# perdoch/hesaff

Measured on AMD Instinct MI355X. Metric: keypoints/sec (descriptors written), 4K grayscale batch, higher is better.
Workload: dtype f32

## Files before the change

hesaff_amd/csrc/capi_impl.h:

```cpp
#pragma once

namespace {

int fail(hesaff_ctx *c, const HsError &e)
{
   if (c) c->err = e.msg; else g_create_error = e.msg;
   return e.code;
}

#define HS_API_BEGIN try {
#define HS_API_END(ctx)                                              \
   }                                                                 \
   catch (const HsError &e) { return fail(ctx, e); }                 \
   catch (const std::exception &e) { return fail(ctx, HsError(HESAFF_ERR_NOMEM, e.what())); } \
   return HESAFF_OK;

void bind_device(hesaff_ctx *c) { HIP_TRY(hipSetDevice(c->device)); }

bool finite_f(float v) { return v == v && v - v == 0.0f; }

void validate_params(const hesaff_params &p)
{
   if (!finite_f(p.threshold) || !finite_f(p.edgeEigenValueRatio) || !finite_f(p.initialSigma) || !finite_f(p.convergenceThreshold) ||
       !finite_f(p.mrSize) || !finite_f(p.maxBinValue))
// ... 113 lines not shown
      if (const char *ov = getenv("HESAFF_OVERLAP")) c->no_overlap = atoi(ov) == 0;
      c->debug = getenv("HESAFF_DEBUG") != nullptr;
#endif
   } catch (const HsError &e) {
      hesaff_destroy(c);
      return fail(nullptr, e);
   } catch (const std::exception &e) {
      hesaff_destroy(c);
      return fail(nullptr, HsError(HESAFF_ERR_NOMEM, e.what()));
   }
   *out = c;
   return HESAFF_OK;
}

void hesaff_destroy(hesaff_ctx *c)
{
   if (!c) return;
   (void)hipSetDevice(c->device);
   if (c->stream) { (void)hipStreamSynchronize(c->stream); }
   DevBuf *bufs[] = {&c->t_smm, &c->t_sift, &c->t_bin0, &c->t_bin1, &c->t_w0, &c->t_w1, &c->t_pyr_taps, &c->t_patch_taps,
                     &c->t_patch_off, &c->t_patch_k, &c->b_gray, &c->b_up, &c->b_L, &c->b_L3, &c->b_R, &c->b_map, &c->b_bitmask, &c->b_prefix,
                     &c->b_blocksums, &c->b_generic, &c->b_counters, &c->b_cand, &c->b_rec_f, &c->b_rec_i, &c->b_rec_w, &c->b_hess_f, &c->b_hess_i,
                     &c->b_aff, &c->b_pw, &c->b_bins, &c->b_rank, &c->b_desc, &c->b_out, &c->b_starts, &c->b_patches,
                     &c->b_stage, &c->b_input, &c->t_mask_idx, &c->t_sgrad_nb, &c->t_sgrad_om, &c->t_vo_rows, &c->t_vo_src, &c->b_rowprefix, &c->b_trows, &c->b_trows2, &c->b_trows3,
                     &c->b_ex_len, &c->b_ex_sums, &c->b_ex_off, &c->b_ex_imgoff, &c->b_ex_starts, &c->b_jcoef[0], &c->b_jcoef[1], &c->b_jplane};
   for (DevBuf *b : bufs) b->release();
   for (hipEvent_t e : c->ev_pool) (void)hipEventDestroy(e);
   {
      hipStream_t all[6] = {c->side_streams[0], c->side_streams[1], c->side_streams[2], c->side_streams[3], c->sift_stream, c->aff_stream};
      for (int i = 0; i < 6; i++) {
         bool seen = all[i] == nullptr || all[i] == c->stream;
         for (int j = 0; j < i; j++) seen = seen || all[j] == all[i];
         if (!seen) (void)hipStreamSynchronize(all[i]);
      }
      for (int i = 0; i < HS_NSIDE; i++) if (c->ev_join[i]) (void)hipEventDestroy(c->ev_join[i]);
   }
   if (c->ev_fork) (void)hipEventDestroy(c->ev_fork);
   if (c->ev_detect_done) (void)hipEventDestroy(c->ev_detect_done);
   if (c->ev_batch_done) (void)hipEventDestroy(c->ev_batch_done);
   for (hipEvent_t e : c->ev_aff) (void)hipEventDestroy(e);
   for (int i = 0; i < HS_NSLOT; i++) {
      if (c->ev_extract_done[i]) (void)hipEventDestroy(c->ev_extract_done[i]);
      if (c->ev_sift_done[i]) (void)hipEventDestroy(c->ev_sift_done[i]);
      c->b_patches2[i].release();
   }
   c->b_siftvec2.release(); c->b_meanvar2.release(); c->b_siftvo2.release();
   if (c->h2d_stream) (void)hipStreamSynchronize(c->h2d_stream);
// ... 749 lines not shown
   Lists s = make_lists(c);
   hipStream_t st = c->stream;
   HIP_TRY(hipMemcpy2DAsync(c->gray.p, (size_t)c->gray.pitch * 4, img, (size_t)cols * 4, (size_t)cols * 4, rows, hipMemcpyHostToDevice, st));
   std::vector<float> x(n), y(n), sc(n);
   std::vector<int32_t> meta(n, 0), P0(n), alive(n);
   for (int i = 0; i < n; i++) { x[i] = kp[3 * i]; y[i] = kp[3 * i + 1]; sc[i] = kp[3 * i + 2]; }
   HIP_TRY(hipMemcpyAsync(s.hl.x, x.data(), (size_t)n * 4, hipMemcpyHostToDevice, st));
   HIP_TRY(hipMemcpyAsync(s.hl.y, y.data(), (size_t)n * 4, hipMemcpyHostToDevice, st));
   HIP_TRY(hipMemcpyAsync(s.hl.s, sc.data(), (size_t)n * 4, hipMemcpyHostToDevice, st));
   HIP_TRY(hipMemcpyAsync(s.hl.meta, meta.data(), (size_t)n * 4, hipMemcpyHostToDevice, st));
   HIP_TRY(hipMemcpyAsync(s.pw.A, A, (size_t)n * 16, hipMemcpyHostToDevice, st));
   HIP_TRY(hipMemsetAsync(s.counters, 0, 64 * 4, st));
   uint32_t nn = (uint32_t)n;
   HIP_TRY(hipMemcpyAsync(s.counters + 3, &nn, 4, hipMemcpyHostToDevice, st));
   hipLaunchKernelGGL(k_prepare_patch_given_A, dim3((n + 255) / 256), dim3(256), 0, st, s.hl, (const uint32_t *)(s.counters + 3), rows, cols,
                      c->consts, c->tables, s.pw);
   c->b_patches.ensure((size_t)n * HS_PATCH_PIX * 4);
   HIP_TRY(hipMemsetAsync(c->b_patches.p, 0, (size_t)n * HS_PATCH_PIX * 4, st));
   unsigned long long large_rows = 0;
   c->batch_max_p = 0;
   for (int i = 0; i < n; i++) {
      const float mrScale = ceilf(sc[i] * c->consts.mrSize);
      const long long P = (mrScale < 1.0e6f) ? 2 * (long long)mrScale + 3 : 0;
      if (P > HS_BIN3_PMAX && P <= c->max_p0 + 2) { large_rows += (unsigned long long)P; c->batch_max_p = std::max(c->batch_max_p, (int)P); }
   }
   if (large_rows > 0xffffffffull) throw HsError(HESAFF_ERR_NOMEM, "too many huge windows in one call");
   run_patch_stage(c, s, c->gray, c->b_patches.as<float>(), 0, (uint32_t)large_rows);
   uint32_t ovf = 0;
   HIP_TRY(hipMemcpyAsync(&ovf, s.counters + 6, 4, hipMemcpyDeviceToHost, st));
   HIP_TRY(hipMemcpyAsync(alive.data(), s.pw.alive, (size_t)n * 4, hipMemcpyDeviceToHost, st));
   if (patches) HIP_TRY(hipMemcpyAsync(patches, c->b_patches.p, (size_t)n * HS_PATCH_PIX * 4, hipMemcpyDeviceToHost, st));
   HIP_TRY(hipStreamSynchronize(st));
   HIP_TRY(hipGetLastError());
   if (ovf) throw HsError(HESAFF_ERR_NOMEM, "large-window row buffer exceeded (internal bound violated)");
   if (rejected) for (int i = 0; i < n; i++) rejected[i] = alive[i] ? 0 : 1;
   HS_API_END(c)
}

int hesaff_stage_sift(hesaff_ctx *c, int n, const float *patches, uint8_t *desc)
{
   if (!c || !patches || !desc || n < 0) return HESAFF_ERR_ARG;
   HS_API_BEGIN
   bind_device(c);
   if (n == 0) return HESAFF_OK;
   const size_t N = (size_t)n;
   const size_t off_alive = N * HS_PATCH_PIX * 4, off_mv = off_alive + N * 4, off_vec = off_mv + N * 8, off_desc = off_vec + N * 128 * 4;
   const size_t off_vo = (off_desc + N * 128 + 63) & ~(size_t)63, total = off_vo + N * HS_VO_PITCH * 8 + 64;
// ... 178 lines not shown
```

hesaff_amd/csrc/kernels_keypoint.h:

```cpp
#pragma once
#include <type_traits>
#include "device_common.h"
#include "kernels_pyramid.h"

struct PlaneTab {
   DPlane L[HS_MAX_OCTAVES][HS_NSCALES];
};

struct KpTables {
   const float *smm_mask;
   const float *sift_mask;
   const int32_t *mask_idx;
   int n_masked;
   const int4 *sgrad_nb;
   const int2 *sgrad_om;
   const int4 *vo_rows;
   const uint16_t *vo_src;
   const int32_t *bin0, *bin1;
   const float *w0, *w1;
   const float *patch_taps;
   const int32_t *patch_tap_off;
   const int32_t *patch_tap_k;
   int max_p0;
};
// ... 204 lines not shown
   hs_affine_groups(
      h_lo, n, tb.smm_mask, k, out, [&](uint32_t h) {
      const int meta = hl.meta[h];
      const int b = meta >> 8, octave = (meta >> 4) & 15, level = (meta >> 2) & 3;
      const DPlane &P = pt.L[octave][level];
      AffKp q;
      q.blur = P.img(b); q.rows = P.rows; q.cols = P.cols; q.pitch = P.pitch;
      q.x = hl.x[h]; q.y = hl.y[h]; q.s = hl.s[h]; q.pd = k.pd0 * (float)(1 << octave);
      return q;
   });
}

__global__ __launch_bounds__(64) void k_affine_stage(DPlane P, const float *__restrict__ kp , int n, KpTables tb, DConsts k,
                                                     AffineOut out)
{
   hs_affine_groups(0u, (uint32_t)n, tb.smm_mask, k, out, [&](uint32_t h) {
      AffKp q;
      q.blur = P.img(0); q.rows = P.rows; q.cols = P.cols; q.pitch = P.pitch;
      q.x = kp[4 * h]; q.y = kp[4 * h + 1]; q.s = kp[4 * h + 2]; q.pd = kp[4 * h + 3];
      return q;
   });
}

#define HS_NBINS 5
#define HS_BIN3_PMAX 512
__host__ __device__ inline int hs_patch_bin(int P) { return P <= 41 ? 0 : (P <= 64 ? 1 : (P <= 128 ? 2 : (P <= HS_BIN3_PMAX ? 3 : 4))); }

struct PatchWork {
   float *A;
   int32_t *P0;
   int32_t *alive;
   uint32_t *bin_count;
   uint32_t *bin_work;
   uint32_t *bin_items;
   uint32_t cap;
};

__device__ __forceinline__ int hs_window_p0(float s, float mrSize)
{
   const float mrScale = ceilf(s * mrSize);
   const int m = (mrScale < 1.0e6f) ? (int)mrScale : 1000000;
   return 2 * m + 1;
}

__global__ __launch_bounds__(256) void k_image_large_rows(HessList hl, const uint32_t *__restrict__ n_ptr, float mrSize, uint32_t *__restrict__ rows, int nimg);

template <bool RECTIFY>
__device__ __forceinline__ void hs_prepare_patch_body(const HessList &hl, uint32_t h_lo, uint32_t n, const AffineOut &aff, int imRows, int imCols,
                                                      const DConsts &k, const KpTables &tb, const PatchWork &pw)
// ... 165 lines not shown
```

hesaff_amd/csrc/kernels_patch.h:

```cpp
#pragma once
#include <type_traits>
#include "kernels_keypoint.h"

#define HS_PATCH_ARR 1684
#define HS_PATCH_PIX_IT 7
#define HS_NEED 82

struct PatchIO {
   DPlane image;
   float *patches;
   uint32_t h_base;
   float *trows;
   const uint32_t *row_prefix;
   uint32_t trows_cap;
   uint32_t *overflow;
};

__device__ __forceinline__ float hs_tap_inside(const HsPlaneBuf &im, float wx, float wy)
{
   const uint32_t off = ((uint32_t)(int)wy * im.pitch + (uint32_t)(int)wx) * 4u;
   wx = __builtin_amdgcn_fractf(wx);
   wy = __builtin_amdgcn_fractf(wy);
   const hs_v2u r0 = __builtin_amdgcn_raw_buffer_load_b64(im.rsrc, (int)off, 0, 0);
   const hs_v2u r1 = __builtin_amdgcn_raw_buffer_load_b64(im.rsrc, (int)off, (int)im.pitch_bytes, 0);
// ... 361 lines not shown
         }
      }
   }
   pa = da;
   pb = db;
}

template <bool PADDED>
__device__ __forceinline__ void hs_resample_reduced_batched(const float *__restrict__ T, int P, float scale, hs_row_taps taps, int r,
                                                            float *s_patch)
{
   const float c0 = (float)(P >> 1);
   for (int idx = threadIdx.x; idx < HS_PATCH_PIX; idx += 256) {
      const int jj = hs_div_small(idx, 1.0f / (float)HS_PATCH), ii = idx - jj * HS_PATCH;
      const int j = jj - (HS_PATCH >> 1), i = ii - (HS_PATCH >> 1);
      const float rx = c0 + (float)j * 0.0f, ry = c0 + (float)j * scale;
      float wx = rx + (float)i * scale, wy = ry + (float)i * 0.0f;
      const float fx = floorf(wx), fy = floorf(wy);
      wx -= fx; wy -= fy;
      const int y0 = min(max((int)fy, 0), P - 2);
      v2f pa, pb;
      hs_colpass4_rows<8, !PADDED>(T, y0, 2 * ii, P - 1, taps, r, pa, pb);
      s_patch[idx] = (1.0f - wy) * ((1.0f - wx) * pa.x + wx * pa.y) + (wy) * ((1.0f - wx) * pb.x + wx * pb.y);
   }
}

__device__ __forceinline__ void hs_resample_chunked(const float *__restrict__ T, int P, float scale, hs_row_taps taps, int r,
                                                    float *__restrict__ s_chunk, int chunk_rows, float *s_patch)
{
   const int tid = threadIdx.x;
   const float c0 = (float)(P >> 1);
   auto y0_of = [&](int jj) {
      const float wy = c0 + (float)(jj - (HS_PATCH >> 1)) * scale;
      return min(max((int)floorf(wy), 0), P - 2);
   };
   for (int jj0 = 0; jj0 < HS_PATCH;) {
      const int ylo = y0_of(jj0) - r;
      int jj1 = jj0;
      while (jj1 + 1 < HS_PATCH && y0_of(jj1 + 1) + r + 2 - ylo <= chunk_rows) jj1++;
      const int nrows = y0_of(jj1) + r + 2 - ylo;
      {
         const v2f *src = reinterpret_cast<const v2f *>(T + ylo * HS_NEED);
         v2f *dst = reinterpret_cast<v2f *>(s_chunk);
         const int n2 = nrows * (HS_NEED / 2);
#pragma unroll 4
         for (int i = tid; i < n2; i += 256) dst[i] = src[i];
      }
      __syncthreads();
      for (int idx = jj0 * HS_PATCH + tid; idx < (jj1 + 1) * HS_PATCH; idx += 256) {
         const int jj = hs_div_small(idx, 1.0f / (float)HS_PATCH), ii = idx - jj * HS_PATCH;
         const int j = jj - (HS_PATCH >> 1), i = ii - (HS_PATCH >> 1);
         const float rx = c0 + (float)j * 0.0f, ry = c0 + (float)j * scale;
         float wx = rx + (float)i * scale, wy = ry + (float)i * 0.0f;
         const float fx = floorf(wx), fy = floorf(wy);
         wx -= fx; wy -= fy;
         const int y0 = min(max((int)fy, 0), P - 2);
         const float *tc = s_chunk + (y0 - ylo) * HS_NEED + 2 * ii;
         auto ld = [&](int dy) { return *reinterpret_cast<const v2f *>(tc + dy * HS_NEED); };
         const v2f q0 = ld(0), q1 = ld(1);
         const float kc = taps[r];
         v2f da = kc * q0, db = kc * q1;
         v2f pj = q1, mj = q0;
#pragma unroll 4
         for (int jt = 1; jt <= r; jt++) {
            const v2f pn = ld(jt + 1), mn = ld(-jt);
            const float kj = taps[r + jt];
            const v2f sa = pj + mn, sb = pn + mj;
            da += kj * sa;
            db += kj * sb;
            pj = pn;
            mj = mn;
         }
         s_patch[idx] = (1.0f - wy) * ((1.0f - wx) * da.x + wx * da.y) + (wy) * ((1.0f - wx) * db.x + wx * db.y);
      }
      __syncthreads();
      jj0 = jj1 + 1;
   }
}

template <int NR, int NB>
__device__ __forceinline__ void hs_gather_slots(const HsPlaneBuf &img, const v2f *rc, const v2f *__restrict__ ctab, float a11, float a21, int half,
                                                int xb, int P, int r, float *__restrict__ srow, int sstride)
{
   const int lane = threadIdx.x & 63, pm = P - 1;
   float v[NR][NB];
#pragma unroll
   for (int it = 0; it < NB; it++) {
      const int xx = min(xb + lane + 64 * it, pm);
      const v2f c = ctab ? ctab[xx] : hs_col_coord(a11, a21, xx - half);
#pragma unroll
      for (int i = 0; i < NR; i++) {
         const v2f w = rc[i] + c;
         v[i][it] = hs_tap_inside(img, w.x, w.y);
      }
   }
#pragma unroll
// ... 137 lines not shown
         a1 = sA[jt + 1]; b1 = sB[jt + 1];
         tA0 += k * a0; tA1 += k * a1;
         tB0 += k * b0; tB1 += k * b1;
      }
      tA2.x = tA0; tA2.y = tA1; tB2.x = tB0; tB2.y = tB1;
      const int yA = rowA ? yy1 : yy0, yB = rowB == 2 ? yy2 : yy1;
      v2f *oA = reinterpret_cast<v2f *>(rowA ? out1 : out0) + colA;
      v2f *oB = reinterpret_cast<v2f *>(rowB == 2 ? out2 : out1) + colB;
      *oA = tA2;
      if (64 + lane < 3 * HS_PATCH) *oB = tB2;
      if (pad_r > 0) {
         if (yA == 0) for (int jr = 1; jr <= pad_r; jr++) oA[-jr * (HS_NEED / 2)] = tA2;
         if (yA == pm) for (int jr = 1; jr <= pad_r; jr++) oA[jr * (HS_NEED / 2)] = tA2;
         if (64 + lane < 3 * HS_PATCH) {
            if (yB == 0) for (int jr = 1; jr <= pad_r; jr++) oB[-jr * (HS_NEED / 2)] = tB2;
            if (yB == pm) for (int jr = 1; jr <= pad_r; jr++) oB[jr * (HS_NEED / 2)] = tB2;
         }
      }
   }
   HS_WAVE_LDS_SYNC();
}

#define HS_MID_PMAX 128
#define HS_MID_SROW 160
#define HS_BIG_SROW 640
#define HS_BIG_TAPS 128
#define HS_MID_RPAD 14
#define HS_BIG_RPAD 57
#define HS_CHUNK_MIN_ROWS 4
#define HS_MID_NIT3_BIG 2
#define HS_MID_NIT3_SMALL 1
#define HS_MID_BLOCKS (256 * 7)
#define HS_BIG_BLOCKS (256 * 8)

template <int PMAX> struct MidGeom {
   static constexpr bool BIG = PMAX > HS_MID_PMAX;
   static constexpr int SROW = BIG ? HS_BIG_SROW : HS_MID_SROW;
   static constexpr int NTAP = BIG ? HS_BIG_TAPS : 32;
   static constexpr int RPAD = BIG ? HS_BIG_RPAD : HS_MID_RPAD;
   static constexpr int CHUNK_MIN = BIG ? 0 : 64;
   static constexpr int SROWS = 12 * SROW > CHUNK_MIN * HS_NEED ? 12 * SROW : CHUNK_MIN * HS_NEED;
   static constexpr int CHUNK_ROWS = SROWS / HS_NEED;
   static constexpr int FLOATS = HS_PATCH_ARR + NTAP + 2 * (PMAX + 2) + SROWS;
};

template <int PMAX>
__global__ __launch_bounds__(256) void k_patch_mid(HessList hl, PatchWork pw, PatchIO io, KpTables tb)
{
   typedef MidGeom<PMAX> GM;
   constexpr int BIN = GM::BIG ? 3 : 2;
   constexpr int NIT = GM::BIG ? 4 : 2;
   constexpr int NIT3 = GM::BIG ? HS_MID_NIT3_BIG : HS_MID_NIT3_SMALL;
   extern __shared__ __attribute__((aligned(16))) float smem[];
   float *s_patch = smem;
   v2f *s_C = reinterpret_cast<v2f *>(s_patch + HS_PATCH_ARR + GM::NTAP);
   float *s_srow = reinterpret_cast<float *>(s_C + (PMAX + 2));
   float *Tp = io.trows + (size_t)blockIdx.x * ((size_t)(PMAX + 2 * GM::RPAD) * HS_NEED);

   const int tid = threadIdx.x, wave = tid >> 6;
   const uint32_t cnt = min(pw.bin_count[BIN], pw.cap);
   const int imPitch = io.image.pitch;

   __shared__ uint32_t s_item;
   for (;;) {
      if (tid == 0) s_item = atomicAdd(pw.bin_work + BIN, 1u);
      __syncthreads();
      const uint32_t wi = (uint32_t)__builtin_amdgcn_readfirstlane((int)s_item);
      if (wi >= cnt) break;
      const uint32_t h = pw.bin_items[(size_t)BIN * pw.cap + wi];
      const int b = hl.meta[h] >> 8;
      const HsPlaneBuf ib = hs_plane_buf(io.image.img(b), io.image.rows, imPitch);
      const float x = hl.x[h], y = hl.y[h];
      const float a11 = pw.A[4 * h], a12 = pw.A[4 * h + 1], a21 = pw.A[4 * h + 2], a22 = pw.A[4 * h + 3];
      const int P0 = pw.P0[h], P = P0 + 2, half = P >> 1;
      const float scale = (float)P0 / (float)HS_PATCH;
      const int K = tb.patch_tap_k[(P0 - 1) >> 1];
      const float *taps_g = tb.patch_taps + tb.patch_tap_off[(P0 - 1) >> 1];
      const hs_row_taps ktap = HS_ROW_TAPS(taps_g);
      for (int m = tid; m < P; m += 256) s_C[m] = hs_col_coord(a11, a21, m - half);
      __syncthreads();
      float *srowA = s_srow + wave * 3 * GM::SROW, *srowB = srowA + GM::SROW;
#pragma unroll 1
      for (int yy = wave; yy < P; yy += 12) {
         const int rr = K >> 1;
         if (yy + 8 < P)
            hs_row_stream3<NIT3>(ib, x, y, a12, a22, P, yy, yy + 4, yy + 8, scale, s_C, ktap, K, srowA, GM::SROW,
                                 Tp + (size_t)(yy + rr) * HS_NEED, Tp + (size_t)(yy + 4 + rr) * HS_NEED, Tp + (size_t)(yy + 8 + rr) * HS_NEED, rr);
         else if (yy + 4 < P)
            hs_row_stream2<NIT>(ib, x, y, a12, a22, P, yy, yy + 4, scale, s_C, ktap, K, srowA, srowB,
                                Tp + (size_t)(yy + (K >> 1)) * HS_NEED, Tp + (size_t)(yy + 4 + (K >> 1)) * HS_NEED, K >> 1);
         else
            hs_row_stream<NIT>(ib, x, y, a11, a12, a21, a22, P, yy, scale, s_C, ktap, K, srowA,
                               Tp + (size_t)(yy + (K >> 1)) * HS_NEED, K >> 1);
      }
      __syncthreads();
      if ((float)(K + 1) + (float)(HS_CHUNK_MIN_ROWS - 1) * scale <= (float)GM::CHUNK_ROWS)
         hs_resample_chunked(Tp + (K >> 1) * HS_NEED, P, scale, ktap, K >> 1, s_srow, GM::CHUNK_ROWS, s_patch);
      else
         hs_resample_reduced_batched<true>(Tp + (K >> 1) * HS_NEED, P, scale, ktap, K >> 1, s_patch);
      __syncthreads();
      for (int i = tid; i < HS_PATCH_PIX; i += 256) {
         float *po = io.patches + (size_t)(h - io.h_base) * HS_PATCH_PIX + i;
         hs_store_nt(po, s_patch[i]);
      }
      __syncthreads();
   }
}

#define HS_LARGE_CHUNK 18
#define HS_LARGE_NIT3 2

__global__ __launch_bounds__(256) void k_patch_large_rows(HessList hl, PatchWork pw, PatchIO io, KpTables tb, int srow_stride, int tap_stride, int nrow,
                                                          int p_lo, int p_hi)
{
   extern __shared__ __attribute__((aligned(16))) float smem[];
   const int wave = __builtin_amdgcn_readfirstlane((int)(threadIdx.x >> 6));
   float *srow = smem + (size_t)wave * (nrow * srow_stride + tap_stride);
   const uint32_t *pre = io.row_prefix;
   const uint32_t n_items = min(pw.bin_count[HS_NBINS - 1], pw.cap);
   if (n_items == 0) return;
   const uint32_t row_hi = pre[n_items];
   if (row_hi > io.trows_cap) {
      if (threadIdx.x == 0 && blockIdx.x == 0) *io.overflow = 1u;
      return;
   }
   const int imPitch = io.image.pitch;
   const uint32_t ntasks = (row_hi + HS_LARGE_CHUNK - 1) / HS_LARGE_CHUNK;
// ... 130 lines not shown
```

hesaff_amd/csrc/pipeline.hip:

```cpp
#include <hip/hip_runtime.h>
#include <algorithm>
#include <atomic>
#include <chrono>
#include <cmath>
#include <cstdio>
#include <cstdlib>
#include <cstring>
#include <string>
#include <vector>
#include <condition_variable>
#include <deque>
#include <future>
#include <map>
#include <memory>
#include <mutex>
#include <thread>

#include "../../include/hesaff_amd.h"
#include "host_tables.h"
#include "kernels_keypoint.h"
#include "kernels_patch.h"
#include "kernels_sift.h"
#include "kernels_pyramid.h"
#include "kernels_export.h"
// ... 106 lines not shown
      if (p) (void)hipFree(p);
      p = nullptr;
      bytes = 0;
   }
   template <class T> T *as() const { return (T *)p; }
};

struct OctGeom {
   int rows, cols, pitch;
   long long word_base;
   int words_per_row;
};

static inline int round_up(int v, int m) { return (v + m - 1) / m * m; }

#define HS_NSIDE 4
#define HS_LARGE_NW 2
#define HS_LARGE_SPLIT 1280
#define HS_AFF_BLOCKS_PER_CU 8
#define HS_GRID_LOC 1024
#define HS_GRID_DED 512
#define HS_GRID_SCAT 1024
#define HS_GRID_PACK 3584
#define HS_MID_CAP 6
#define HS_BIG_CAP 4
#define HS_OVERSUB 128u
#define HS_NSLOT 3
struct StreamSet { hipStream_t comp[4] = {nullptr, nullptr, nullptr, nullptr}; hipStream_t h2d = nullptr, d2h = nullptr; };
static std::mutex g_sets_mu;
static std::map<int, std::vector<StreamSet>> g_idle_sets;
static bool take_stream_set(int device, StreamSet &out)
{
   std::lock_guard<std::mutex> lk(g_sets_mu);
   std::vector<StreamSet> &v = g_idle_sets[device];
   if (v.empty()) return false;
   out = v.back();
   v.pop_back();
   return true;
}
static void give_stream_set(int device, const StreamSet &s)
{
   std::lock_guard<std::mutex> lk(g_sets_mu);
   g_idle_sets[device].push_back(s);
}

struct hesaff_ctx {
   hesaff_params par;
   int device = 0;
// ... 117 lines not shown
   hipStream_t h2d_stream = nullptr, d2h_stream = nullptr;
   hipEvent_t ev_exp[2][4] = {{nullptr, nullptr, nullptr, nullptr}, {nullptr, nullptr, nullptr, nullptr}};
   float export_ms = 0.0f; int32_t export_rows = 0;
   hipEvent_t ev_h2d[2] = {nullptr, nullptr}, ev_in_free[2] = {nullptr, nullptr}, ev_out_ready[2] = {nullptr, nullptr}, ev_d2h[2] = {nullptr, nullptr};
   struct HostSmall {
      void *p = nullptr; size_t bytes = 0;
      void *ensure(size_t need)
      {
         if (need > bytes) {
            if (p) (void)hipHostFree(p);
            p = nullptr; bytes = 0;
            const size_t cap = std::max<size_t>(need * 2, 4096);
            if (hipHostMalloc(&p, cap, hipHostMallocDefault) != hipSuccess) { p = nullptr; throw HsError(HESAFF_ERR_NOMEM, "hipHostMalloc failed (small result block)"); }
            bytes = cap;
         }
         return p;
      }
      void release() { if (p) (void)hipHostFree(p); p = nullptr; bytes = 0; }
   } h_small_end, h_small_mid, h_small_exp;
   struct HStarts {
      int32_t *q = nullptr;
      int32_t *data() const { return q; }
   } h_starts;
   DevBuf t_mask_idx, t_sgrad_nb, t_sgrad_om, t_vo_rows, t_vo_src, b_rowprefix, b_trows, b_trows2, b_trows3;
   DevBuf b_jcoef[2], b_jplane;
   DevBuf b_ex_len, b_ex_sums, b_ex_off, b_ex_imgoff, b_ex_starts;
   size_t rows_lds_set = 0;
   int n_cu = 256;
   uint32_t g_small0 = 256 * 6, g_small1 = 256 * 4, g_mid = HS_MID_BLOCKS, g_big = HS_BIG_BLOCKS, g_lfin = 256 * 4, g_shist = 256 * 32;
   uint32_t sgrad_grid = 256 * 32;
   uint32_t trows_rows = 4u << 20;

   hesaff_timings tm;
   int profiling = 0;
   int out_format = HESAFF_OUT_TEXT;
   int resume = 0;
   int pool_priority = -1;
   int stage_threads = 4;
   hipStream_t side_streams[HS_NSIDE] = {nullptr, nullptr, nullptr, nullptr};
   hipStream_t sift_stream = nullptr;
   hipStream_t aff_stream = nullptr;
   hipEvent_t ev_detect_done = nullptr, ev_batch_done = nullptr;
   std::vector<hipEvent_t> ev_aff;
   hipEvent_t ev_extract_done[HS_NSLOT] = {}, ev_sift_done[HS_NSLOT] = {};
   DevBuf b_patches2[HS_NSLOT];
   DevBuf b_siftvec2, b_meanvar2, b_siftvo2;
   hipEvent_t ev_fork = nullptr, ev_join[HS_NSIDE] = {nullptr, nullptr, nullptr, nullptr};
   bool fast_pyramid = false;
   bool no_overlap = false;
   bool debug = false;

   std::vector<hipEvent_t> ev_pool;
// ... 120 lines not shown
   t.bin0 = c->t_bin0.as<int32_t>(); t.bin1 = c->t_bin1.as<int32_t>();
   t.w0 = c->t_w0.as<float>(); t.w1 = c->t_w1.as<float>();
   t.patch_taps = c->t_patch_taps.as<float>(); t.patch_tap_off = c->t_patch_off.as<int32_t>(); t.patch_tap_k = c->t_patch_k.as<int32_t>();
   t.max_p0 = c->max_p0;
   t.mask_idx = c->t_mask_idx.as<int32_t>();
   t.sgrad_nb = c->t_sgrad_nb.as<int4>(); t.sgrad_om = c->t_sgrad_om.as<int2>();
   t.vo_rows = c->t_vo_rows.as<int4>(); t.vo_src = c->t_vo_src.as<uint16_t>();
   t.n_masked = c->n_masked;
}

DPlane make_plane(float *p, int rows, int cols, int pitch)
{
   DPlane d;
   d.p = p; d.rows = rows; d.cols = cols; d.pitch = pitch; d.img_stride = (long long)rows * pitch;
   return d;
}

template <class KERNEL> void set_dyn_lds(KERNEL kern, size_t lds)
{
   HIP_TRY(hipFuncSetAttribute((const void *)kern, hipFuncAttributeMaxDynamicSharedMemorySize, (int)lds));
}

size_t small_extract_lds_bytes(int bin) { return (size_t)(bin == 0 ? SmallGeom<0>::FLOATS : SmallGeom<1>::FLOATS) * 4; }
size_t mid_lds_bytes() { return (size_t)MidGeom<HS_MID_PMAX>::FLOATS * 4; }
size_t big_lds_bytes() { return (size_t)MidGeom<HS_BIN3_PMAX>::FLOATS * 4; }

constexpr size_t HS_LDS_PER_CU = 160 * 1024;
struct LargeGeom { int srow_stride, tap_stride; size_t lds; };
LargeGeom large_geom(int pmax)
{
   LargeGeom g;
   g.srow_stride = round_up((int)(pmax * 1.23) + 16, 64);
   g.tap_stride = round_up((int)(pmax * 0.22) + 8, 64);
   g.lds = (size_t)4 * (g.srow_stride + g.tap_stride) * 4;
   return g;
}

template <class KERNEL> uint32_t resident_grid(hesaff_ctx *c, KERNEL kern, int threads, size_t dyn_lds, uint32_t fallback_per_cu)
{
   int nb = 0;
   if (hipOccupancyMaxActiveBlocksPerMultiprocessor(&nb, (const void *)kern, threads, dyn_lds) != hipSuccess || nb < 1) {
      (void)hipGetLastError();
      nb = (int)fallback_per_cu;
   }
   return (uint32_t)c->n_cu * (uint32_t)nb;
}

void set_kernel_attrs(hesaff_ctx *c)
{
   set_dyn_lds(k_patch_extract_small<0>, small_extract_lds_bytes(0));
   set_dyn_lds(k_patch_extract_small<1>, small_extract_lds_bytes(1));
   set_dyn_lds(k_patch_mid<HS_MID_PMAX>, mid_lds_bytes());
   set_dyn_lds(k_patch_mid<HS_BIN3_PMAX>, big_lds_bytes());
   hipDeviceProp_t prop;
   HIP_TRY(hipGetDeviceProperties(&prop, c->device));
   c->n_cu = std::max(1, prop.multiProcessorCount);
   c->g_small0 = resident_grid(c, k_patch_extract_small<0>, 256, small_extract_lds_bytes(0), 6);
   c->g_small1 = resident_grid(c, k_patch_extract_small<1>, 256, small_extract_lds_bytes(1), 4);
   c->g_mid = std::min<uint32_t>(resident_grid(c, k_patch_mid<HS_MID_PMAX>, 256, mid_lds_bytes(), HS_MID_CAP), HS_MID_BLOCKS);
   c->g_big = std::min<uint32_t>(resident_grid(c, k_patch_mid<HS_BIN3_PMAX>, 256, big_lds_bytes(), HS_BIG_CAP), HS_BIG_BLOCKS);
   c->g_lfin = resident_grid(c, k_patch_large_finish, 256, 0, 4);
   c->g_shist = resident_grid(c, k_sift_hist, 64, 0, 32);
   c->sgrad_grid = (uint32_t)c->n_cu * 32u;
   c->g_small0 *= HS_OVERSUB; c->g_small1 *= HS_OVERSUB; c->g_shist *= HS_OVERSUB;
}

void plan_buffers(hesaff_ctx *c, int B, int H, int W);
void plan(hesaff_ctx *c, int B, int H, int W)
{
   try {
      plan_buffers(c, B, H, W);
   } catch (const HsError &e) {
      if (e.code == HESAFF_ERR_NOMEM) {
         DevBuf *bufs[] = {&c->b_gray, &c->b_up, &c->b_L, &c->b_L3, &c->b_R, &c->b_map, &c->b_bitmask, &c->b_prefix, &c->b_blocksums, &c->b_cand,
                           &c->b_rec_f, &c->b_rec_i, &c->b_rec_w, &c->b_hess_f, &c->b_hess_i, &c->b_aff, &c->b_pw, &c->b_bins, &c->b_rank, &c->b_desc,
                           &c->b_out, &c->b_starts};
         (void)hipStreamSynchronize(c->stream);
         for (DevBuf *b : bufs) b->release();
         c->map_clean = false;
      }
      throw;
   }
}
// ... 68 lines not shown
   c->b_counters.ensure(64 * 4);
   {
      const unsigned long long waves0 = (unsigned long long)((PW + EXM_STRIP - 1) / EXM_STRIP) * (unsigned long long)(PH / 32 + 1) * (unsigned long long)B;
      const unsigned long long cc = (unsigned long long)cap + (unsigned long long)cap / 8 + HS_CAND_BLOCK * waves0;
      if (cc > 0xfffffff0ull) throw HsError(HESAFF_ERR_ARG, "batch too large for 32-bit candidate indices");
      c->cand_cap = (uint32_t)cc;
      c->b_cand.ensure((size_t)cc * sizeof(CandRec));
   }
   c->b_rec_f.ensure(cap * 4 * 4);
   c->b_rec_i.ensure(cap * 4 * 4);
   c->b_rec_w.ensure(cap * 8);
   c->b_hess_f.ensure(cap * 4 * 4);
   c->b_hess_i.ensure(cap * 2 * 4);
   c->b_aff.ensure(cap * 6 * 4);
   c->b_pw.ensure(cap * 6 * 4);
   c->b_bins.ensure(cap * HS_NBINS * 4);
   c->b_rank.ensure((cap + 1) * 4);
   c->b_desc.ensure(cap * 128);
   c->b_out.ensure(cap * sizeof(KeyRec));
   c->b_starts.ensure(((size_t)(B + 1) * 3 + 2) * 4);
   const int max_p0 = (int)std::floor(std::sqrt((double)W * (double)H)) + 3;
   ensure_patch_taps(c, max_p0);
   refresh_tables_struct(c);
   c->b_trows2.ensure((size_t)HS_MID_BLOCKS * (HS_MID_PMAX + 2 * HS_MID_RPAD) * HS_NEED * 4);
   c->b_trows3.ensure((size_t)HS_BIG_BLOCKS * (HS_BIN3_PMAX + 2 * HS_BIG_RPAD) * HS_NEED * 4);
   {
      const LargeGeom lg = large_geom(c->max_p0 + 2);
      if (lg.lds / 4 > HS_LDS_PER_CU) throw HsError(HESAFF_ERR_ARG, "image too large for the large-window row kernel (sqrt(width x height) above about 27900)");
      const size_t want = std::min<size_t>(lg.lds + (size_t)8 * lg.srow_stride * 4, HS_LDS_PER_CU);
      if (want > c->rows_lds_set) {
         set_dyn_lds(k_patch_large_rows, want);
         c->rows_lds_set = want;
      }
   }
   c->B = B; c->H = H; c->W = W;
}

template <class LOAD> void exclusive_scan(hesaff_ctx *c, LOAD load, long long n, uint32_t *out, uint32_t *total)
{
   if (n <= 0) { HIP_TRY(hipMemsetAsync(total, 0, 4, c->stream)); return; }
   const int nb = (int)((n + SCAN_BLOCK - 1) / SCAN_BLOCK);
   uint32_t *bs = c->b_blocksums.as<uint32_t>();
   hipLaunchKernelGGL(k_scan_reduce<LOAD>, dim3(nb), dim3(256), 0, c->stream, load, n, bs);
   hipLaunchKernelGGL(k_scan_sums, dim3(1), dim3(256), 0, c->stream, bs, nb, total);
   hipLaunchKernelGGL(k_scan_down<LOAD>, dim3(nb), dim3(256), 0, c->stream, load, n, bs, out);
}

struct StageTimer {
// ... 117 lines not shown
   io.h_base = h_base;
   if (c->fast_pyramid && pt) {
      hipStream_t s0 = st;
      const bool forked = c->side_streams[0] && !c->no_overlap;
      if (forked) {
         HIP_TRY(hipEventRecord(c->ev_fork, st));
         HIP_TRY(hipStreamWaitEvent(c->side_streams[0], c->ev_fork, 0));
         s0 = c->side_streams[0];
      }
      hipLaunchKernelGGL(k_patch_extract_small<0>, dim3(c->g_small0), dim3(256), small_extract_lds_bytes(0), s0, s.hl, s.pw, io, c->tables);
      if (forked) HIP_TRY(hipEventRecord(c->ev_join[0], s0));
      hipLaunchKernelGGL(k_patch_pyramid, dim3((uint32_t)c->n_cu * 32u), dim3(256), 0, st, s.hl, s.pw, io, *pt, (int)c->oct.size(), c->consts.pd0, 1);
      if (forked) HIP_TRY(hipStreamWaitEvent(st, c->ev_join[0], 0));
      return;
   }
   hipStream_t s0 = st, s1 = st, s2 = st, s3 = st;
   const bool forked = c->side_streams[0] && !c->no_overlap;
   if (forked) {
      HIP_TRY(hipEventRecord(c->ev_fork, st));
      for (int i = 0; i < HS_NSIDE; i++) HIP_TRY(hipStreamWaitEvent(c->side_streams[i], c->ev_fork, 0));
      s0 = c->side_streams[0]; s1 = c->side_streams[1]; s2 = c->side_streams[2]; s3 = c->side_streams[3];
   }
   {
      PatchIO io2 = io;
      io2.trows = c->b_trows2.as<float>();
      PatchIO io3 = io;
      io3.trows = c->b_trows3.as<float>();
      hipLaunchKernelGGL(k_patch_extract_small<0>, dim3(c->g_small0), dim3(256), small_extract_lds_bytes(0), s0, s.hl, s.pw, io, c->tables);
      hipLaunchKernelGGL(k_patch_extract_small<1>, dim3(c->g_small1), dim3(256), small_extract_lds_bytes(1), s1, s.hl, s.pw, io, c->tables);
      hipLaunchKernelGGL(k_patch_mid<HS_MID_PMAX>, dim3(c->g_mid), dim3(256), mid_lds_bytes(), s2, s.hl, s.pw, io2, c->tables);
      hipLaunchKernelGGL(k_patch_mid<HS_BIN3_PMAX>, dim3(c->g_big), dim3(256), big_lds_bytes(), s3, s.hl, s.pw, io3, c->tables);
   }
   if (large_rows_bound > 0) {
      const uint32_t rows_cap = std::max(large_rows_bound, c->trows_rows);
      c->b_trows.ensure((size_t)rows_cap * HS_NEED * 4);
      c->b_rowprefix.ensure(((size_t)c->cap + 1) * 4);
      const int pmax = std::min(c->max_p0 + 2, std::max(HS_BIN3_PMAX + 1, (c->batch_max_p > 0 ? c->batch_max_p : c->max_p0 + 2)));
      io.trows = c->b_trows.as<float>();
      io.row_prefix = c->b_rowprefix.as<uint32_t>();
      io.trows_cap = rows_cap;
      io.overflow = s.counters + 6;
      hipLaunchKernelGGL(k_large_prefix, dim3(1), dim3(256), 0, st, s.pw, c->b_rowprefix.as<uint32_t>());
      auto launch_rows = [&](int p_lo, int p_hi) {
         const LargeGeom lg = large_geom(std::min(c->max_p0 + 2, (p_hi + 255) / 256 * 256));
         const size_t wave1 = lg.lds / 4;
         const size_t wave3 = wave1 + (size_t)2 * lg.srow_stride * 4;
         const int nrow = wave3 * 6 <= HS_LDS_PER_CU ? 3 : 1;
         const size_t per_wave = nrow == 3 ? wave3 : wave1;
         uint32_t nw = 4;
         while (nw > 1 && per_wave * nw > HS_LDS_PER_CU) nw >>= 1;
         if (nw == 4 && (HS_LDS_PER_CU / (per_wave * 2)) * 2 > (HS_LDS_PER_CU / (per_wave * 4)) * 4) nw = 2;
         if (nrow == 3) nw = std::min<uint32_t>(nw, HS_LARGE_NW);
         const uint32_t gblocks = std::min<uint32_t>((large_rows_bound + nw * HS_LARGE_CHUNK - 1) / (nw * HS_LARGE_CHUNK), 256 * 16 * (4 / nw));
         hipLaunchKernelGGL(k_patch_large_rows, dim3(gblocks), dim3(64 * nw), per_wave * nw, st, s.hl, s.pw, io, c->tables, lg.srow_stride, lg.tap_stride, nrow,
                            p_lo, std::min(p_hi, 0x7ffffff0));
      };
      if (pmax > HS_LARGE_SPLIT) { launch_rows(0, HS_LARGE_SPLIT); launch_rows(HS_LARGE_SPLIT, pmax); }
      else launch_rows(0, pmax);
      hipLaunchKernelGGL(k_patch_large_finish, dim3(c->g_lfin), dim3(256), 0, st, s.pw, io, c->tables);
   }
// ... 407 lines not shown
```

Before: 38.95 million.

## Keep mid-window row planes resident in LDS and split mid bin

Mid-size patch windows (65..128) are split into two bins at 113, each compiled with its own LDS geometry. The transformed row plane now lives in LDS instead of a global scratch buffer, and the final resample is done straight from LDS to the output patch, skipping the global round trip and the staging patch array. The cost is much larger LDS per block, so fewer blocks fit per CU. Both mid kernels now run back to back on one side stream instead of overlapping.

```diff
diff --git a/hesaff_amd/csrc/capi_impl.h b/hesaff_amd/csrc/capi_impl.h
--- a/hesaff_amd/csrc/capi_impl.h
+++ b/hesaff_amd/csrc/capi_impl.h
@@ -159,7 +159,7 @@
                      &c->t_patch_off, &c->t_patch_k, &c->b_gray, &c->b_up, &c->b_L, &c->b_L3, &c->b_R, &c->b_map, &c->b_bitmask, &c->b_prefix,
                      &c->b_blocksums, &c->b_generic, &c->b_counters, &c->b_cand, &c->b_rec_f, &c->b_rec_i, &c->b_rec_w, &c->b_hess_f, &c->b_hess_i,
                      &c->b_aff, &c->b_pw, &c->b_bins, &c->b_rank, &c->b_desc, &c->b_out, &c->b_starts, &c->b_patches,
-                     &c->b_stage, &c->b_input, &c->t_mask_idx, &c->t_sgrad_nb, &c->t_sgrad_om, &c->t_vo_rows, &c->t_vo_src, &c->b_rowprefix, &c->b_trows, &c->b_trows2, &c->b_trows3,
+                     &c->b_stage, &c->b_input, &c->t_mask_idx, &c->t_sgrad_nb, &c->t_sgrad_om, &c->t_vo_rows, &c->t_vo_src, &c->b_rowprefix, &c->b_trows, &c->b_trows4,
                      &c->b_ex_len, &c->b_ex_sums, &c->b_ex_off, &c->b_ex_imgoff, &c->b_ex_starts, &c->b_jcoef[0], &c->b_jcoef[1], &c->b_jplane};
    for (DevBuf *b : bufs) b->release();
    for (hipEvent_t e : c->ev_pool) (void)hipEventDestroy(e);
@@ -955,7 +955,7 @@
    for (int i = 0; i < n; i++) {
       const float mrScale = ceilf(sc[i] * c->consts.mrSize);
       const long long P = (mrScale < 1.0e6f) ? 2 * (long long)mrScale + 3 : 0;
-      if (P > HS_BIN3_PMAX && P <= c->max_p0 + 2) { large_rows += (unsigned long long)P; c->batch_max_p = std::max(c->batch_max_p, (int)P); }
+      if (P > HS_BIG_PMAX && P <= c->max_p0 + 2) { large_rows += (unsigned long long)P; c->batch_max_p = std::max(c->batch_max_p, (int)P); }
    }
    if (large_rows > 0xffffffffull) throw HsError(HESAFF_ERR_NOMEM, "too many huge windows in one call");
    run_patch_stage(c, s, c->gray, c->b_patches.as<float>(), 0, (uint32_t)large_rows);
diff --git a/hesaff_amd/csrc/kernels_keypoint.h b/hesaff_amd/csrc/kernels_keypoint.h
--- a/hesaff_amd/csrc/kernels_keypoint.h
+++ b/hesaff_amd/csrc/kernels_keypoint.h
@@ -250,9 +250,10 @@
    });
 }
 
-#define HS_NBINS 5
-#define HS_BIN3_PMAX 512
-__host__ __device__ inline int hs_patch_bin(int P) { return P <= 41 ? 0 : (P <= 64 ? 1 : (P <= 128 ? 2 : (P <= HS_BIN3_PMAX ? 3 : 4))); }
+#define HS_NBINS 6
+#define HS_BIG_PMAX 512
+#define HS_MID_SPLIT 113
+__host__ __device__ constexpr int hs_patch_bin(int P) { return P <= 41 ? 0 : (P <= 64 ? 1 : (P <= HS_MID_SPLIT ? 2 : (P <= 128 ? 3 : (P <= HS_BIG_PMAX ? 4 : 5)))); }
 
 struct PatchWork {
    float *A;
diff --git a/hesaff_amd/csrc/kernels_patch.h b/hesaff_amd/csrc/kernels_patch.h
--- a/hesaff_amd/csrc/kernels_patch.h
+++ b/hesaff_amd/csrc/kernels_patch.h
@@ -407,6 +407,41 @@
       v2f pa, pb;
       hs_colpass4_rows<8, !PADDED>(T, y0, 2 * ii, P - 1, taps, r, pa, pb);
       s_patch[idx] = (1.0f - wy) * ((1.0f - wx) * pa.x + wx * pa.y) + (wy) * ((1.0f - wx) * pb.x + wx * pb.y);
+   }
+}
+
+__device__ __forceinline__ float hs_colpass_lds(const float *__restrict__ tc, hs_row_taps taps, int r, float wx, float wy)
+{
+   auto ld = [&](int dy) { return *reinterpret_cast<const v2f *>(tc + dy * HS_NEED); };
+   const v2f q0 = ld(0), q1 = ld(1);
+   const float kc = taps[r];
+   v2f da = kc * q0, db = kc * q1;
+   v2f pj = q1, mj = q0;
+#pragma unroll 4
+   for (int jt = 1; jt <= r; jt++) {
+      const v2f pn = ld(jt + 1), mn = ld(-jt);
+      const float kj = taps[r + jt];
+      const v2f sa = pj + mn, sb = pn + mj;
+      da += kj * sa;
+      db += kj * sb;
+      pj = pn;
+      mj = mn;
+   }
+   return (1.0f - wy) * ((1.0f - wx) * da.x + wx * da.y) + (wy) * ((1.0f - wx) * db.x + wx * db.y);
+}
+
+__device__ __forceinline__ void hs_resample_resident(const float *__restrict__ T, int P, float scale, hs_row_taps taps, int r, float *__restrict__ out)
+{
+   const float c0 = (float)(P >> 1);
+   for (int idx = threadIdx.x; idx < HS_PATCH_PIX; idx += 256) {
+      const int jj = hs_div_small(idx, 1.0f / (float)HS_PATCH), ii = idx - jj * HS_PATCH;
+      const int j = jj - (HS_PATCH >> 1), i = ii - (HS_PATCH >> 1);
+      const float rx = c0 + (float)j * 0.0f, ry = c0 + (float)j * scale;
+      float wx = rx + (float)i * scale, wy = ry + (float)i * 0.0f;
+      const float fx = floorf(wx), fy = floorf(wy);
+      wx -= fx; wy -= fy;
+      const int y0 = min(max((int)fy, 0), P - 2);
+      hs_store_nt(out + idx, hs_colpass_lds(T + y0 * HS_NEED + 2 * ii, taps, r, wx, wy));
    }
 }
 
@@ -440,23 +475,7 @@
          const float fx = floorf(wx), fy = floorf(wy);
          wx -= fx; wy -= fy;
          const int y0 = min(max((int)fy, 0), P - 2);
-         const float *tc = s_chunk + (y0 - ylo) * HS_NEED + 2 * ii;
-         auto ld = [&](int dy) { return *reinterpret_cast<const v2f *>(tc + dy * HS_NEED); };
-         const v2f q0 = ld(0), q1 = ld(1);
-         const float kc = taps[r];
-         v2f da = kc * q0, db = kc * q1;
-         v2f pj = q1, mj = q0;
-#pragma unroll 4
-         for (int jt = 1; jt <= r; jt++) {
-            const v2f pn = ld(jt + 1), mn = ld(-jt);
-            const float kj = taps[r + jt];
-            const v2f sa = pj + mn, sb = pn + mj;
-            da += kj * sa;
-            db += kj * sb;
-            pj = pn;
-            mj = mn;
-         }
-         s_patch[idx] = (1.0f - wy) * ((1.0f - wx) * da.x + wx * da.y) + (wy) * ((1.0f - wx) * db.x + wx * db.y);
+         s_patch[idx] = hs_colpass_lds(s_chunk + (y0 - ylo) * HS_NEED + 2 * ii, taps, r, wx, wy);
       }
       __syncthreads();
       jj0 = jj1 + 1;
@@ -640,40 +659,40 @@
 }
 
 #define HS_MID_PMAX 128
-#define HS_MID_SROW 160
 #define HS_BIG_SROW 640
-#define HS_BIG_TAPS 128
-#define HS_MID_RPAD 14
 #define HS_BIG_RPAD 57
 #define HS_CHUNK_MIN_ROWS 4
 #define HS_MID_NIT3_BIG 2
 #define HS_MID_NIT3_SMALL 1
-#define HS_MID_BLOCKS (256 * 7)
 #define HS_BIG_BLOCKS (256 * 8)
+
+constexpr int hs_mid_rpad(int pmax) { return ((int)(9.0 * (pmax - 2) / 41.0 + 1.01) | 1) >> 1; }
 
 template <int PMAX> struct MidGeom {
    static constexpr bool BIG = PMAX > HS_MID_PMAX;
-   static constexpr int SROW = BIG ? HS_BIG_SROW : HS_MID_SROW;
-   static constexpr int NTAP = BIG ? HS_BIG_TAPS : 32;
-   static constexpr int RPAD = BIG ? HS_BIG_RPAD : HS_MID_RPAD;
-   static constexpr int CHUNK_MIN = BIG ? 0 : 64;
-   static constexpr int SROWS = 12 * SROW > CHUNK_MIN * HS_NEED ? 12 * SROW : CHUNK_MIN * HS_NEED;
-   static constexpr int CHUNK_ROWS = SROWS / HS_NEED;
-   static constexpr int FLOATS = HS_PATCH_ARR + NTAP + 2 * (PMAX + 2) + SROWS;
+   static constexpr int BIN = BIG ? 4 : (PMAX > HS_MID_SPLIT ? 3 : 2);
+   static constexpr int RPAD = BIG ? HS_BIG_RPAD : hs_mid_rpad(PMAX);
+   static constexpr int SROW = BIG ? HS_BIG_SROW : (PMAX + 2 * RPAD + 4 + 3) & ~3;
+   static constexpr int CHUNK_ROWS = 12 * SROW / HS_NEED;
+   static constexpr int PLANE = BIG ? 0 : (PMAX + 2 * RPAD) * HS_NEED;
+   static constexpr int FLOATS = (BIG ? HS_PATCH_ARR : 0) + 2 * (PMAX + 2) + 12 * SROW + PLANE;
+   static_assert(BIG || hs_patch_bin(PMAX) == BIN, "a launch's largest window lies in its bin");
+   static_assert((2 * (PMAX + 2) + 12 * SROW) % 2 == 0 && HS_PATCH_ARR % 2 == 0, "pairs must stay 8-byte aligned");
 };
+static_assert(hs_mid_rpad(HS_MID_PMAX) == 14 && hs_mid_rpad(HS_BIG_PMAX) <= HS_BIG_RPAD, "K / 2 of the largest windows");
 
 template <int PMAX>
 __global__ __launch_bounds__(256) void k_patch_mid(HessList hl, PatchWork pw, PatchIO io, KpTables tb)
 {
    typedef MidGeom<PMAX> GM;
-   constexpr int BIN = GM::BIG ? 3 : 2;
+   constexpr int BIN = GM::BIN;
    constexpr int NIT = GM::BIG ? 4 : 2;
    constexpr int NIT3 = GM::BIG ? HS_MID_NIT3_BIG : HS_MID_NIT3_SMALL;
    extern __shared__ __attribute__((aligned(16))) float smem[];
    float *s_patch = smem;
-   v2f *s_C = reinterpret_cast<v2f *>(s_patch + HS_PATCH_ARR + GM::NTAP);
+   v2f *s_C = reinterpret_cast<v2f *>(smem + (GM::BIG ? HS_PATCH_ARR : 0));
    float *s_srow = reinterpret_cast<float *>(s_C + (PMAX + 2));
-   float *Tp = io.trows + (size_t)blockIdx.x * ((size_t)(PMAX + 2 * GM::RPAD) * HS_NEED);
+   float *Tp = GM::BIG ? io.trows + (size_t)blockIdx.x * ((size_t)(PMAX + 2 * GM::RPAD) * HS_NEED) : s_srow + 12 * GM::SROW;
 
    const int tid = threadIdx.x, wave = tid >> 6;
    const uint32_t cnt = min(pw.bin_count[BIN], pw.cap);
@@ -698,29 +717,30 @@
       for (int m = tid; m < P; m += 256) s_C[m] = hs_col_coord(a11, a21, m - half);
       __syncthreads();
       float *srowA = s_srow + wave * 3 * GM::SROW, *srowB = srowA + GM::SROW;
+      const int rr = K >> 1;
 #pragma unroll 1
       for (int yy = wave; yy < P; yy += 12) {
-         const int rr = K >> 1;
+         float *t0 = Tp + (yy + rr) * HS_NEED;
          if (yy + 8 < P)
             hs_row_stream3<NIT3>(ib, x, y, a12, a22, P, yy, yy + 4, yy + 8, scale, s_C, ktap, K, srowA, GM::SROW,
-                                 Tp + (size_t)(yy + rr) * HS_NEED, Tp + (size_t)(yy + 4 + rr) * HS_NEED, Tp + (size_t)(yy + 8 + rr) * HS_NEED, rr);
+                                 t0, t0 + 4 * HS_NEED, t0 + 8 * HS_NEED, rr);
          else if (yy + 4 < P)
-            hs_row_stream2<NIT>(ib, x, y, a12, a22, P, yy, yy + 4, scale, s_C, ktap, K, srowA, srowB,
-                                Tp + (size_t)(yy + (K >> 1)) * HS_NEED, Tp + (size_t)(yy + 4 + (K >> 1)) * HS_NEED, K >> 1);
+            hs_row_stream2<NIT>(ib, x, y, a12, a22, P, yy, yy + 4, scale, s_C, ktap, K, srowA, srowB, t0, t0 + 4 * HS_NEED, rr);
          else
-            hs_row_stream<NIT>(ib, x, y, a11, a12, a21, a22, P, yy, scale, s_C, ktap, K, srowA,
-                               Tp + (size_t)(yy + (K >> 1)) * HS_NEED, K >> 1);
-      }
-      __syncthreads();
+            hs_row_stream<NIT>(ib, x, y, a11, a12, a21, a22, P, yy, scale, s_C, ktap, K, srowA, t0, rr);
+      }
+      __syncthreads();
+      float *out = io.patches + (size_t)(h - io.h_base) * HS_PATCH_PIX;
+      if (!GM::BIG) {
+         hs_resample_resident(Tp + rr * HS_NEED, P, scale, ktap, rr, out);
+         continue;
+      }
       if ((float)(K + 1) + (float)(HS_CHUNK_MIN_ROWS - 1) * scale <= (float)GM::CHUNK_ROWS)
-         hs_resample_chunked(Tp + (K >> 1) * HS_NEED, P, scale, ktap, K >> 1, s_srow, GM::CHUNK_ROWS, s_patch);
+         hs_resample_chunked(Tp + rr * HS_NEED, P, scale, ktap, rr, s_srow, GM::CHUNK_ROWS, s_patch);
       else
-         hs_resample_reduced_batched<true>(Tp + (K >> 1) * HS_NEED, P, scale, ktap, K >> 1, s_patch);
-      __syncthreads();
-      for (int i = tid; i < HS_PATCH_PIX; i += 256) {
-         float *po = io.patches + (size_t)(h - io.h_base) * HS_PATCH_PIX + i;
-         hs_store_nt(po, s_patch[i]);
-      }
+         hs_resample_reduced_batched<true>(Tp + rr * HS_NEED, P, scale, ktap, rr, s_patch);
+      __syncthreads();
+      for (int i = tid; i < HS_PATCH_PIX; i += 256) hs_store_nt(out + i, s_patch[i]);
       __syncthreads();
    }
 }
diff --git a/hesaff_amd/csrc/pipeline.hip b/hesaff_amd/csrc/pipeline.hip
--- a/hesaff_amd/csrc/pipeline.hip
+++ b/hesaff_amd/csrc/pipeline.hip
@@ -152,8 +152,8 @@
 #define HS_GRID_DED 512
 #define HS_GRID_SCAT 1024
 #define HS_GRID_PACK 3584
-#define HS_MID_CAP 6
-#define HS_BIG_CAP 4
+#define HS_MID_FALLBACK 2
+#define HS_BIG_FALLBACK 4
 #define HS_OVERSUB 128u
 #define HS_NSLOT 3
 struct StreamSet { hipStream_t comp[4] = {nullptr, nullptr, nullptr, nullptr}; hipStream_t h2d = nullptr, d2h = nullptr; };
@@ -317,12 +317,12 @@
       int32_t *q = nullptr;
       int32_t *data() const { return q; }
    } h_starts;
-   DevBuf t_mask_idx, t_sgrad_nb, t_sgrad_om, t_vo_rows, t_vo_src, b_rowprefix, b_trows, b_trows2, b_trows3;
+   DevBuf t_mask_idx, t_sgrad_nb, t_sgrad_om, t_vo_rows, t_vo_src, b_rowprefix, b_trows, b_trows4;
    DevBuf b_jcoef[2], b_jplane;
    DevBuf b_ex_len, b_ex_sums, b_ex_off, b_ex_imgoff, b_ex_starts;
    size_t rows_lds_set = 0;
    int n_cu = 256;
-   uint32_t g_small0 = 256 * 6, g_small1 = 256 * 4, g_mid = HS_MID_BLOCKS, g_big = HS_BIG_BLOCKS, g_lfin = 256 * 4, g_shist = 256 * 32;
+   uint32_t g_small0 = 256 * 6, g_small1 = 256 * 4, g_mid_lo = 256 * 3, g_mid_hi = 256 * 2, g_big = HS_BIG_BLOCKS, g_lfin = 256 * 4, g_shist = 256 * 32;
    uint32_t sgrad_grid = 256 * 32;
    uint32_t trows_rows = 4u << 20;
 
@@ -489,8 +489,7 @@
 }
 
 size_t small_extract_lds_bytes(int bin) { return (size_t)(bin == 0 ? SmallGeom<0>::FLOATS : SmallGeom<1>::FLOATS) * 4; }
-size_t mid_lds_bytes() { return (size_t)MidGeom<HS_MID_PMAX>::FLOATS * 4; }
-size_t big_lds_bytes() { return (size_t)MidGeom<HS_BIN3_PMAX>::FLOATS * 4; }
+template <int PMAX> constexpr size_t mid_lds_bytes() { return (size_t)MidGeom<PMAX>::FLOATS * 4; }
 
 constexpr size_t HS_LDS_PER_CU = 160 * 1024;
 struct LargeGeom { int srow_stride, tap_stride; size_t lds; };
@@ -517,15 +516,17 @@
 {
    set_dyn_lds(k_patch_extract_small<0>, small_extract_lds_bytes(0));
    set_dyn_lds(k_patch_extract_small<1>, small_extract_lds_bytes(1));
-   set_dyn_lds(k_patch_mid<HS_MID_PMAX>, mid_lds_bytes());
-   set_dyn_lds(k_patch_mid<HS_BIN3_PMAX>, big_lds_bytes());
+   set_dyn_lds(k_patch_mid<HS_MID_SPLIT>, mid_lds_bytes<HS_MID_SPLIT>());
+   set_dyn_lds(k_patch_mid<HS_MID_PMAX>, mid_lds_bytes<HS_MID_PMAX>());
+   set_dyn_lds(k_patch_mid<HS_BIG_PMAX>, mid_lds_bytes<HS_BIG_PMAX>());
    hipDeviceProp_t prop;
    HIP_TRY(hipGetDeviceProperties(&prop, c->device));
    c->n_cu = std::max(1, prop.multiProcessorCount);
    c->g_small0 = resident_grid(c, k_patch_extract_small<0>, 256, small_extract_lds_bytes(0), 6);
    c->g_small1 = resident_grid(c, k_patch_extract_small<1>, 256, small_extract_lds_bytes(1), 4);
-   c->g_mid = std::min<uint32_t>(resident_grid(c, k_patch_mid<HS_MID_PMAX>, 256, mid_lds_bytes(), HS_MID_CAP), HS_MID_BLOCKS);
-   c->g_big = std::min<uint32_t>(resident_grid(c, k_patch_mid<HS_BIN3_PMAX>, 256, big_lds_bytes(), HS_BIG_CAP), HS_BIG_BLOCKS);
+   c->g_mid_lo = resident_grid(c, k_patch_mid<HS_MID_SPLIT>, 256, mid_lds_bytes<HS_MID_SPLIT>(), HS_MID_FALLBACK);
+   c->g_mid_hi = resident_grid(c, k_patch_mid<HS_MID_PMAX>, 256, mid_lds_bytes<HS_MID_PMAX>(), HS_MID_FALLBACK);
+   c->g_big = std::min<uint32_t>(resident_grid(c, k_patch_mid<HS_BIG_PMAX>, 256, mid_lds_bytes<HS_BIG_PMAX>(), HS_BIG_FALLBACK), HS_BIG_BLOCKS);
    c->g_lfin = resident_grid(c, k_patch_large_finish, 256, 0, 4);
    c->g_shist = resident_grid(c, k_sift_hist, 64, 0, 32);
    c->sgrad_grid = (uint32_t)c->n_cu * 32u;
@@ -640,8 +641,7 @@
    const int max_p0 = (int)std::floor(std::sqrt((double)W * (double)H)) + 3;
    ensure_patch_taps(c, max_p0);
    refresh_tables_struct(c);
-   c->b_trows2.ensure((size_t)HS_MID_BLOCKS * (HS_MID_PMAX + 2 * HS_MID_RPAD) * HS_NEED * 4);
-   c->b_trows3.ensure((size_t)HS_BIG_BLOCKS * (HS_BIN3_PMAX + 2 * HS_BIG_RPAD) * HS_NEED * 4);
+   c->b_trows4.ensure((size_t)HS_BIG_BLOCKS * (HS_BIG_PMAX + 2 * HS_BIG_RPAD) * HS_NEED * 4);
    {
       const LargeGeom lg = large_geom(c->max_p0 + 2);
       if (lg.lds / 4 > HS_LDS_PER_CU) throw HsError(HESAFF_ERR_ARG, "image too large for the large-window row kernel (sqrt(width x height) above about 27900)");
@@ -805,20 +805,19 @@
       s0 = c->side_streams[0]; s1 = c->side_streams[1]; s2 = c->side_streams[2]; s3 = c->side_streams[3];
    }
    {
-      PatchIO io2 = io;
-      io2.trows = c->b_trows2.as<float>();
-      PatchIO io3 = io;
-      io3.trows = c->b_trows3.as<float>();
+      PatchIO io4 = io;
+      io4.trows = c->b_trows4.as<float>();
       hipLaunchKernelGGL(k_patch_extract_small<0>, dim3(c->g_small0), dim3(256), small_extract_lds_bytes(0), s0, s.hl, s.pw, io, c->tables);
       hipLaunchKernelGGL(k_patch_extract_small<1>, dim3(c->g_small1), dim3(256), small_extract_lds_bytes(1), s1, s.hl, s.pw, io, c->tables);
-      hipLaunchKernelGGL(k_patch_mid<HS_MID_PMAX>, dim3(c->g_mid), dim3(256), mid_lds_bytes(), s2, s.hl, s.pw, io2, c->tables);
-      hipLaunchKernelGGL(k_patch_mid<HS_BIN3_PMAX>, dim3(c->g_big), dim3(256), big_lds_bytes(), s3, s.hl, s.pw, io3, c->tables);
+      hipLaunchKernelGGL(k_patch_mid<HS_MID_SPLIT>, dim3(c->g_mid_lo), dim3(256), mid_lds_bytes<HS_MID_SPLIT>(), s2, s.hl, s.pw, io, c->tables);
+      hipLaunchKernelGGL(k_patch_mid<HS_MID_PMAX>, dim3(c->g_mid_hi), dim3(256), mid_lds_bytes<HS_MID_PMAX>(), s2, s.hl, s.pw, io, c->tables);
+      hipLaunchKernelGGL(k_patch_mid<HS_BIG_PMAX>, dim3(c->g_big), dim3(256), mid_lds_bytes<HS_BIG_PMAX>(), s3, s.hl, s.pw, io4, c->tables);
    }
    if (large_rows_bound > 0) {
       const uint32_t rows_cap = std::max(large_rows_bound, c->trows_rows);
       c->b_trows.ensure((size_t)rows_cap * HS_NEED * 4);
       c->b_rowprefix.ensure(((size_t)c->cap + 1) * 4);
-      const int pmax = std::min(c->max_p0 + 2, std::max(HS_BIN3_PMAX + 1, (c->batch_max_p > 0 ? c->batch_max_p : c->max_p0 + 2)));
+      const int pmax = std::min(c->max_p0 + 2, std::max(HS_BIG_PMAX + 1, (c->batch_max_p > 0 ? c->batch_max_p : c->max_p0 + 2)));
       io.trows = c->b_trows.as<float>();
       io.row_prefix = c->b_rowprefix.as<uint32_t>();
       io.trows_cap = rows_cap;
```

Result: no change. 38.63 million (median of 3 runs) (-0.8%).
